# arielgabizon/barretenberg

Hardware: AMD Instinct MI355X
Metric: BN254 G1 MSM points/sec at n=2^20 (Fr NTT elems/sec in 'ntt') (higher is better)
Workload: dtype u32x9 (256-bit Montgomery, 29-bit limbs)

## Files before the change

barretenberg_amd/csrc/msm.hip:

```cpp
#include <hip/hip_runtime.h>

#include <algorithm>
#include <mutex>
#include <stdint.h>
#include <stdio.h>
#include <stdlib.h>
#include <string.h>
#include <vector>

#include "bbgpu_internal.h"
#include "g1.hpp"
#include "g1_quad.hpp"
#include "host_g1.hpp"

namespace bbgpu {

using Fr = FrP;
#define FRONT_PRIO() __builtin_amdgcn_s_setprio(2)
constexpr int TAIL_PRIO = 3;
constexpr int SCALAR_BITS = 254;
constexpr int MSM_MAX_C = 16;
constexpr int MSM_THREADS = 256;

__device__ __forceinline__ void ld8(const uint32_t* p, uint32_t (&w)[8])
{
    const uint4* q = reinterpret_cast<const uint4*>(p);
    uint4 a = q[0], b = q[1];
    w[0] = a.x; w[1] = a.y; w[2] = a.z; w[3] = a.w;
    w[4] = b.x; w[5] = b.y; w[6] = b.z; w[7] = b.w;
}
__device__ __forceinline__ void ld16(const uint32_t* p, uint32_t (&w)[16])
{
    const uint4* q = reinterpret_cast<const uint4*>(p);
#pragma unroll
    for (int i = 0; i < 4; i++) {
        uint4 a = q[i];
        w[4 * i] = a.x; w[4 * i + 1] = a.y; w[4 * i + 2] = a.z; w[4 * i + 3] = a.w;
    }
}
__device__ __forceinline__ void st32(uint32_t* p, const uint32_t (&w)[32])
{
    uint4* q = reinterpret_cast<uint4*>(p);
#pragma unroll
    for (int i = 0; i < 8; i++) q[i] = make_uint4(w[4 * i], w[4 * i + 1], w[4 * i + 2], w[4 * i + 3]);
}
__device__ __forceinline__ void ld32(const uint32_t* p, uint32_t (&w)[32])
{
    const uint4* q = reinterpret_cast<const uint4*>(p);
#pragma unroll
    for (int i = 0; i < 8; i++) {
        uint4 a = q[i];
        w[4 * i] = a.x; w[4 * i + 1] = a.y; w[4 * i + 2] = a.z; w[4 * i + 3] = a.w;
    }
}

struct WinLayout {
    uint16_t off[66];
};
static WinLayout make_layout(int c, bool balanced)
{
    WinLayout LO{};
    const int W = msm_num_windows(c);
    if (!balanced) {
        for (int w = 0; w <= W; w++) LO.off[w] = (uint16_t)(c * w);
        return LO;
    }
    const int base = SCALAR_BITS / W, rem = SCALAR_BITS - base * W;
    int bit = 0;
    for (int w = 0; w < W; w++) {
        LO.off[w] = (uint16_t)bit;
        bit += base + (w < rem ? 1 : 0);
    }
    LO.off[W] = (uint16_t)bit;
    return LO;
}
__global__ void srs_convert_kernel(const uint32_t* __restrict__ table, uint32_t* __restrict__ srs, uint32_t n, uint32_t stride_words)
{
    const uint32_t i = blockIdx.x * blockDim.x + threadIdx.x;
    if (i >= n) return;
    uint32_t w[16];
    ld16(table + (size_t)i * stride_words, w);
    AffineV<2> a;
    load_affine_m256(a, w);
    uint32_t o[16];
    store_affine_m261(o, a.x, a.y);
    uint4* q = reinterpret_cast<uint4*>(srs + (size_t)i * 16);
#pragma unroll
    for (int k = 0; k < 4; k++) q[k] = make_uint4(o[4 * k], o[4 * k + 1], o[4 * k + 2], o[4 * k + 3]);
}

__global__ void srs_export_kernel(const uint32_t* __restrict__ srs, uint32_t* __restrict__ table, uint32_t n)
{
    const uint32_t i = blockIdx.x * blockDim.x + threadIdx.x;
    if (i >= n) return;
    uint32_t w[16];
    ld16(srs + (size_t)i * 16, w);
    AffineV<1> a;
    load_affine_m261(a, w);
    uint32_t o[8];
    uint32_t* dst = table + (size_t)i * 32;
    to_canonical(m261_to_m256<Fq>(a.x), o);
    for (int k = 0; k < 8; k++) dst[k] = o[k];
    to_canonical(m261_to_m256<Fq>(a.y), o);
    for (int k = 0; k < 8; k++) dst[8 + k] = o[k];
    auto bx = mul(a.x, fe_from<Fq>(Fq::BETA));
    to_canonical(m261_to_m256<Fq>(bx), o);
    for (int k = 0; k < 8; k++) dst[16 + k] = o[k];
    to_canonical(m261_to_m256<Fq>(weak(neg(a.y))), o);
// ... 116 lines not shown
    } else {
        return dg[i];
    }
}
template <class DT> __device__ __forceinline__ void load_digits8(const DT* __restrict__ dg, const unsigned long long* __restrict__ sg, uint32_t i8, int (&d)[8])
{
    const uint4 q = *reinterpret_cast<const uint4*>(dg + i8);
    const uint32_t w[4] = { q.x, q.y, q.z, q.w };
    if constexpr (DigitTraits<DT>::wide) {
        const uint32_t sb = reinterpret_cast<const uint8_t*>(sg)[i8 >> 3];
#pragma unroll
        for (int k = 0; k < 8; k++) {
            const int u = (int)((w[k >> 1] >> (16 * (k & 1))) & 0xffffu);
            d[k] = ((sb >> k) & 1u) ? -u - 1 : u;
        }
    } else {
#pragma unroll
        for (int k = 0; k < 8; k++) d[k] = (int)(int16_t)(w[k >> 1] >> (16 * (k & 1)));
    }
}
template <class DT> __global__ void __launch_bounds__(MSM_THREADS) msm_digits_kernel(ScalarSets sets, DT* __restrict__ digits_all, unsigned long long* __restrict__ signs_all,
                                                               uint32_t n, WinLayout LO, uint32_t num_windows, uint32_t wb, uint32_t we)
{
    FRONT_PRIO();
    const uint32_t i = blockIdx.x * blockDim.x + threadIdx.x;
    if (i >= n) return;
    const uint32_t* __restrict__ scalars = sets.p[blockIdx.y];
    DT* __restrict__ digits = digits_all + (size_t)blockIdx.y * num_windows * n;
    const uint32_t s64 = (n + 63) >> 6;
    unsigned long long* __restrict__ signs = signs_all + (size_t)blockIdx.y * num_windows * s64;
    uint32_t w[8], k[9];
    ld8(scalars + (size_t)i * 8, w);
    to_canonical(exact_limbs(mul(unpack<Fr>(w), fe_from<Fr>(Fr::M256_TO_PLAIN))), w);
#pragma unroll
    for (int j = 0; j < 8; j++) k[j] = w[j];
    k[8] = 0;
    uint32_t carry = 0;
    for (uint32_t win = 0; win < we; win++) {
        const uint32_t bit = LO.off[win], sz = LO.off[win + 1] - bit, j = bit >> 5, s = bit & 31;
        const uint32_t half = 1u << (sz - 1), mask = (1u << sz) - 1;
        uint32_t v = 0;
        if (j < 8) {
            v = k[j] >> s;
            if (s + sz > 32) v |= k[j + 1] << (32 - s);
        }
        v = (v & mask) + carry;
        carry = (win + 1 < num_windows && v >= half) ? 1u : 0u;
        const int32_t d = (int32_t)v - (int32_t)(carry << sz);
        if (win >= wb) {
            if constexpr (DigitTraits<DT>::wide) {
                const unsigned long long neg = __ballot(d < 0);
                digits[(size_t)win * n + i] = (DT)(d < 0 ? -d - 1 : d);
                if ((threadIdx.x & 63u) == 0) signs[(size_t)win * s64 + (i >> 6)] = neg;
            } else {
                digits[(size_t)win * n + i] = (DT)d;
            }
        }
    }
}

constexpr int SORT_THREADS = 1024;
constexpr uint32_t SORT_MAX_LB = 7;
constexpr uint32_t SORTB_MAX_PARTS = 8;
constexpr uint32_t SORTB_SPLIT_MIN = 1u << 16;

__device__ __forceinline__ bool wave_keys_heavy(bool valid, uint32_t key)
{
    const uint64_t vm = __ballot(valid);
    if (!vm) return false;
    const uint32_t k0 = __builtin_amdgcn_readlane(key, __ffsll((unsigned long long)vm) - 1);
    return 4 * __popcll(__ballot(valid && key == k0)) >= __popcll(vm);
}
__device__ __forceinline__ uint32_t lds_inc_dedup(uint32_t* ctr, uint32_t key, bool heavy)
{
    if (!heavy) return atomicAdd(&ctr[key], 1u);
    const uint32_t lane = __lane_id();
    uint64_t todo = __ballot(1);
    uint32_t res = 0;
    for (int it = 0; it < 4 && todo; it++) {
        const int leader = __ffsll((unsigned long long)todo) - 1;
        const uint32_t kk = __builtin_amdgcn_readlane(key, leader);
// ... 50 lines not shown
    }
    __syncthreads();
    if (threadIdx.x < bins) histA[((size_t)wl * slices + s) * bins + threadIdx.x] = lh[threadIdx.x];
}

__global__ void __launch_bounds__(SORT_THREADS) sortA_colscan_kernel(uint32_t* __restrict__ histA, uint32_t* __restrict__ bintot, uint32_t bins,
                                                                   uint32_t slices)
{
    FRONT_PRIO();
    const uint32_t wl = blockIdx.y, lane = threadIdx.x & 63;
    const uint32_t bin = blockIdx.x * (SORT_THREADS / 64) + (threadIdx.x >> 6);
    if (bin >= bins) return;
    uint32_t* H = histA + (size_t)wl * slices * bins + bin;
    const uint32_t spp = (slices + 63) / 64;
    const uint32_t s0 = min(slices, lane * spp), s1 = min(slices, s0 + spp);
    uint32_t sum = 0;
    for (uint32_t s = s0; s < s1; s++) sum += H[(size_t)s * bins];
    uint32_t incl = sum;
#pragma unroll
    for (int off = 1; off < 64; off <<= 1) {
        const uint32_t v = __shfl_up(incl, off);
        if ((int)lane >= off) incl += v;
    }
    uint32_t run = incl - sum;
    for (uint32_t s = s0; s < s1; s++) {
        const uint32_t cnt = H[(size_t)s * bins];
        H[(size_t)s * bins] = run;
        run += cnt;
    }
    if (lane == 63) bintot[(size_t)wl * bins + bin] = incl;
}
__global__ void __launch_bounds__(SORT_THREADS) sortA_scan_kernel(const uint32_t* __restrict__ bintot, uint32_t* __restrict__ binstart,
                                                                uint32_t* __restrict__ totals, uint32_t bins, uint32_t* __restrict__ solo_bases,
                                                                uint32_t* __restrict__ solo_gstart_end)
{
    FRONT_PRIO();
    __shared__ uint32_t part[SORT_THREADS];
    const uint32_t wl = blockIdx.x, t = threadIdx.x;
    const uint32_t mine = t < bins ? bintot[(size_t)wl * bins + t] : 0;
    part[t] = mine;
    __syncthreads();
    for (uint32_t off = 1; off < SORT_THREADS; off <<= 1) {
        uint32_t v = t >= off ? part[t - off] : 0;
        __syncthreads();
        part[t] += v;
        __syncthreads();
    }
    if (t < bins) binstart[(size_t)wl * bins + t] = part[t] - mine;
    if (t == SORT_THREADS - 1) {
        totals[wl] = part[SORT_THREADS - 1];
        if (solo_bases) {
            solo_bases[0] = 0;
            solo_bases[1] = part[SORT_THREADS - 1];
            solo_gstart_end[0] = part[SORT_THREADS - 1];
            solo_gstart_end[1] = 0xffffffffu;
        }
    }
}
__global__ void sort_bases_kernel(const uint32_t* __restrict__ totals, uint32_t* __restrict__ bases, uint32_t* __restrict__ gstart_end, uint32_t nw)
{
    FRONT_PRIO();
    if (threadIdx.x == 0 && blockIdx.x == 0) {
        uint32_t run = 0;
        for (uint32_t w = 0; w < nw; w++) {
            bases[w] = run;
            run += totals[w];
        }
        bases[nw] = run;
        gstart_end[0] = run;
        gstart_end[1] = 0xffffffffu;
    }
}


template <class DT> __global__ void __launch_bounds__(SORT_THREADS) __attribute__((amdgpu_num_vgpr(32))) sortA_scatter_kernel(const DT* __restrict__ digits, const unsigned long long* __restrict__ signs, const uint32_t* __restrict__ cursorsA,
                                                                   const uint32_t* __restrict__ binstart, const uint32_t* __restrict__ bases,
                                                                   uint32_t* __restrict__ tmp, uint32_t n, uint32_t bins, uint32_t lb,
                                                                   uint32_t slices, uint32_t slice_len, uint32_t win0, uint32_t wpg,
                                                                   uint32_t idx_stride, uint32_t windows_per_job, uint32_t first_i0, uint32_t last_i1, uint32_t blo, uint32_t bcnt)
{
    FRONT_PRIO();
    __shared__ uint32_t lc[SORT_THREADS];
    const uint32_t s = blockIdx.x, wl = blockIdx.y;
    if (threadIdx.x < bins)
        lc[threadIdx.x] = cursorsA[((size_t)wl * slices + s) * bins + threadIdx.x] + binstart[(size_t)wl * bins + threadIdx.x] + bases[wl];
    __syncthreads();
    const uint32_t lo = s * slice_len, hi = min(n, lo + slice_len);
    const uint32_t lomask = (1u << lb) - 1;
    const uint32_t s64 = (n + 63) >> 6;
    if ((n & 7u) == 0) {
        const uint32_t lo8 = lo & ~7u, bpw = lo < hi ? (((hi + 7u) & ~7u) - lo8) >> 3 : 0u;
        for (uint32_t u = threadIdx.x; u < wpg * bpw; u += SORT_THREADS) {
            const uint32_t k = u / bpw, i8 = lo8 + (u - k * bpw) * 8;
            const uint32_t wabs = win0 + wl * wpg + k;
            const uint32_t row = (wabs % windows_per_job) * idx_stride;
            const uint32_t klo = (k == 0) ? max(lo, first_i0) : lo, khi = (k + 1 == wpg) ? min(hi, last_i1) : hi;
            int d[8];
            load_digits8<DT>(digits + (size_t)wabs * n, signs + (size_t)wabs * s64, i8, d);
#pragma unroll
            for (int j = 0; j < 8; j++) {
                if (d[j] && i8 + j >= klo && i8 + j < khi) {
                    const uint32_t b = (uint32_t)((d[j] < 0 ? -d[j] : d[j]) - 1);
                    if (b - blo < bcnt) {
// ... 289 lines not shown
    const u32x4* q = reinterpret_cast<const u32x4*>(p);
    r.q0 = q[0]; r.q1 = q[1]; r.q2 = q[2]; r.q3 = q[3];
#endif
}
__device__ __forceinline__ void row_land(RowRegs& r, uint32_t (&w)[16])
{
#if defined(__HIP_DEVICE_COMPILE__)
    __builtin_amdgcn_s_waitcnt(0x0f70);
    asm volatile("" : "+v"(r.q0), "+v"(r.q1), "+v"(r.q2), "+v"(r.q3));
#endif
#pragma unroll
    for (int i = 0; i < 4; i++) { w[i] = r.q0[i]; w[4 + i] = r.q1[i]; w[8 + i] = r.q2[i]; w[12 + i] = r.q3[i]; }
}
__device__ __forceinline__ void value_landed(uint32_t& v)
{
#if defined(__HIP_DEVICE_COMPILE__)
    asm volatile("" : "+v"(v));
#endif
}
__device__ __forceinline__ void operand_done(Fe<Fq, 1, 1>& x, Fe<Fq, 1, 2>& y)
{
#if defined(__HIP_DEVICE_COMPILE__)
    asm volatile("" : "+v"(x.d[0]), "+v"(x.d[1]), "+v"(x.d[2]), "+v"(x.d[3]), "+v"(x.d[4]), "+v"(x.d[5]), "+v"(x.d[6]), "+v"(x.d[7]), "+v"(x.d[8]));
    asm volatile("" : "+v"(y.d[0]), "+v"(y.d[1]), "+v"(y.d[2]), "+v"(y.d[3]), "+v"(y.d[4]), "+v"(y.d[5]), "+v"(y.d[6]), "+v"(y.d[7]), "+v"(y.d[8]));
#endif
}
constexpr int RAW_WORDS = 4 * NL;
constexpr uint32_t HEAVY_WGS = 256;
constexpr uint32_t HEAVY_IDS = 1 + HEAVY_WGS;
static_assert(MSM_THREADS == (int)HEAVY_WGS, "heavy-bucket queue header is cleared / combined by one lane per K4h workgroup");

__global__ void __launch_bounds__(MSM_THREADS) msm_accumulate_kernel(const uint32_t* __restrict__ srs, const uint32_t* __restrict__ sorted,
                                                                   const uint32_t* __restrict__ gstart, uint32_t* __restrict__ partials,
                                                                   uint32_t total_buckets, uint32_t ch, uint32_t prio, uint32_t* __restrict__ heavy_counter)
{
    if (heavy_counter && blockIdx.x == 0) {
        heavy_counter[threadIdx.x] = 0;
        if (threadIdx.x == 0) heavy_counter[MSM_THREADS] = 0;
    }
    if (prio == 1) __builtin_amdgcn_s_setprio(1);
    else if (prio == 2) __builtin_amdgcn_s_setprio(2);
    const uint32_t t = blockIdx.x * blockDim.x + threadIdx.x;
    const uint32_t M = gstart[total_buckets];
    const uint32_t p0 = t * ch;
    if (p0 >= M) return;
    const uint32_t p1 = min(M, p0 + ch);
    uint32_t lo = 0, hi = total_buckets;
    while (hi - lo > 1) {
        const uint32_t mid = (lo + hi) >> 1;
        if (gstart[mid] <= p0) lo = mid; else hi = mid;
    }
    uint32_t b = lo;
    uint32_t next_end = gstart[b + 1];
    Xyzz acc;
    set_infinity(acc);
    uint32_t after_next = gstart[min(b + 2, total_buckets + 1)];
    bool acc_inf = true;
    uint32_t v = sorted[p0];
    uint32_t vn = sorted[p0 + 1 < p1 ? p0 + 1 : p0];
    RowRegs row;
    uint32_t w[16];
    row_request(row, srs + (size_t)(v & 0x7fffffffu) * 16);
    Fe<Fq, 1, 1> px;
    Fe<Fq, 1, 2> py;
    row_land(row, w);
    load_affine_m261_signed(px, py, w, (v >> 31) != 0);
    operand_done(px, py);
    row_request(row, srs + (size_t)(vn & 0x7fffffffu) * 16);
    uint32_t e = p0;
    uint32_t trips = ch;
    do {
        const uint32_t vnn = sorted[min(e + 2, p1 - 1)];
        const bool start = (e == next_end) || acc_inf;
        if (start) {
            if (e == next_end) {
                store_raw(partials + (size_t)(b + t) * RAW_WORDS, acc);
// ... 47 lines not shown
}
#define TAIL_OCC __attribute__((amdgpu_waves_per_eu(4, 4)))
constexpr int FOLD_T = 256;
constexpr int FOLD_LDS_WORDS = (FOLD_T / 2) * RAW_WORDS;
__device__ __forceinline__ void wg_tree_sum(Xyzz& acc, uint32_t* sh, uint32_t T, uint32_t t)
{
    constexpr uint32_t STRIDE = FOLD_T / 2;
    for (uint32_t half = T >> 1; half >= 1; half >>= 1) {
        if (t >= half && t < 2 * half) {
#pragma unroll
            for (int i = 0; i < NL; i++) {
                sh[(0 * NL + i) * STRIDE + t - half] = acc.x.d[i];
                sh[(1 * NL + i) * STRIDE + t - half] = acc.y.d[i];
                sh[(2 * NL + i) * STRIDE + t - half] = acc.zz.d[i];
                sh[(3 * NL + i) * STRIDE + t - half] = acc.zzz.d[i];
            }
        }
        __syncthreads();
        if (t < half) {
            Xyzz q, r;
#pragma unroll
            for (int i = 0; i < NL; i++) {
                q.x.d[i] = sh[(0 * NL + i) * STRIDE + t];
                q.y.d[i] = sh[(1 * NL + i) * STRIDE + t];
                q.zz.d[i] = sh[(2 * NL + i) * STRIDE + t];
                q.zzz.d[i] = sh[(3 * NL + i) * STRIDE + t];
            }
            add(r, acc, q);
            acc = r;
        }
        __syncthreads();
    }
}
__global__ void __launch_bounds__(MSM_THREADS) TAIL_OCC msm_merge_kernel(const uint32_t* __restrict__ gstart, const uint32_t* __restrict__ partials,
                                                              uint32_t* __restrict__ buckets, uint32_t* __restrict__ heavy, uint32_t bucket_begin, uint32_t total_buckets,
                                                              uint32_t ch, uint32_t MERGE_LIGHT, uint32_t logG)
{
    __builtin_amdgcn_s_setprio(TAIL_PRIO);
    const uint32_t t = blockIdx.x * blockDim.x + threadIdx.x;
    const uint32_t G = 1u << logG, b = bucket_begin + (t >> logG), j = t & (G - 1);
    if (b >= total_buckets) return;
    const uint32_t s = gstart[b], e = gstart[b + 1];
    Xyzz acc;
    set_infinity(acc);
    if (e > s) {
        const uint32_t t0 = s / ch, t1 = (e - 1) / ch;
        if (t1 - t0 >= MERGE_LIGHT) {
            if (j == 0) heavy[HEAVY_IDS + atomicAdd(&heavy[0], 1u)] = b;
            return;
        }
        for (uint32_t k = t0 + j; k <= t1; k += G) {
            Xyzz q, r;
            load_raw(q, partials + (size_t)(b + k) * RAW_WORDS);
            add(r, acc, q);
            acc = r;
        }
    }
    for (uint32_t off = G >> 1; off >= 1; off >>= 1) {
        const Xyzz o = shfl_down_xyzz(acc, off);
        if (j < off) {
            Xyzz r;
            add(r, acc, o);
            acc = r;
        }
    }
    if (j == 0) {
        uint32_t o[32];
        store_xyzz(o, acc);
        st32(buckets + (size_t)b * 32, o);
    }
}
__global__ void __launch_bounds__(MSM_THREADS) TAIL_OCC msm_merge_heavy_kernel(const uint32_t* __restrict__ gstart, const uint32_t* __restrict__ partials,
                                                                    uint32_t* __restrict__ buckets, uint32_t* __restrict__ heavy, uint32_t ch, uint32_t* __restrict__ hpart)
{
    __builtin_amdgcn_s_setprio(TAIL_PRIO);
    __shared__ uint32_t sh[FOLD_LDS_WORDS];
    __shared__ uint32_t last_flag;
    const uint32_t count = heavy[0];
    const uint32_t K = count ? gridDim.x / count : 0;
    if (K < 2) {
        for (uint32_t item = blockIdx.x; item < count; item += gridDim.x) {
            const uint32_t b = heavy[HEAVY_IDS + item];
            const uint32_t s = gstart[b], e = gstart[b + 1];
            const uint32_t t0 = s / ch, t1 = (e - 1) / ch;
            Xyzz acc;
            set_infinity(acc);
            for (uint32_t t = t0 + threadIdx.x; t <= t1; t += MSM_THREADS) {
                Xyzz q, r;
                load_raw(q, partials + (size_t)(b + t) * RAW_WORDS);
                add(r, acc, q);
                acc = r;
            }
            __syncthreads();
            wg_tree_sum(acc, sh, MSM_THREADS, threadIdx.x);
            if (threadIdx.x == 0) {
                uint32_t o[32];
                store_xyzz(o, acc);
                st32(buckets + (size_t)b * 32, o);
            }
        }
        return;
    }
    const uint32_t item = blockIdx.x / K, sub = blockIdx.x - item * K;
    if (item >= count) return;
    const uint32_t b = heavy[HEAVY_IDS + item];
    const uint32_t s = gstart[b], e = gstart[b + 1];
    const uint32_t t0 = s / ch, t1 = (e - 1) / ch, total = t1 - t0 + 1;
// ... 57 lines not shown
    constexpr uint32_t NW = T / 64;
    const uint32_t waves = min(NW, (active + 15) / 16);
    if (waves <= 1) return acc;
    if (lane < 4) {
#pragma unroll
        for (int i = 0; i < NL; i++) sh[(wave * 4 + l) * NL + i] = acc.d[i];
    }
    __syncthreads();
    if (wave == 0) {
        acc = quad_zero();
        if (qd < NW) {
#pragma unroll
            for (int i = 0; i < NL; i++) acc.d[i] = sh[(qd * 4 + l) * NL + i];
        }
        for (uint32_t off = NW >> 1; off >= 1; off >>= 1) {
            if (off >= waves) continue;
            FqN o;
#pragma unroll
            for (int i = 0; i < NL; i++) o.d[i] = __shfl_down(acc.d[i], off * 4);
            if (qd < off) acc = quad_add(acc, o, l);
        }
    }
    return acc;
}
__device__ __forceinline__ void quad_store8(uint32_t* dst8, const uint32_t (&w)[8])
{
    uint4* q = reinterpret_cast<uint4*>(dst8);
    q[0] = make_uint4(w[0], w[1], w[2], w[3]);
    q[1] = make_uint4(w[4], w[5], w[6], w[7]);
}

__global__ void __launch_bounds__(MSM_THREADS) TAIL_OCC msm_merge_quad_kernel(const uint32_t* __restrict__ gstart, const uint32_t* __restrict__ partials,
                                                                   uint32_t* __restrict__ buckets, uint32_t* __restrict__ heavy, uint32_t bucket_begin, uint32_t total_buckets,
                                                                   uint32_t ch, uint32_t MERGE_LIGHT, uint32_t logQ)
{
    __builtin_amdgcn_s_setprio(TAIL_PRIO);
    const uint32_t t = blockIdx.x * blockDim.x + threadIdx.x, l = t & 3, quad = t >> 2;
    const uint32_t Q = 1u << logQ, b = bucket_begin + (quad >> logQ), j = quad & (Q - 1);
    if (b >= total_buckets) return;
    const uint32_t s = gstart[b], e = gstart[b + 1];
    FqN acc = quad_zero();
    if (e > s) {
        const uint32_t t0 = s / ch, t1 = (e - 1) / ch;
        if (t1 - t0 >= MERGE_LIGHT) {
            if (j == 0 && l == 0) heavy[HEAVY_IDS + atomicAdd(&heavy[0], 1u)] = b;
            return;
        }
        uint32_t k = t0 + j;
        if (k <= t1) {
            const uint32_t* src = partials + (size_t)(b + k) * RAW_WORDS + NL * l;
#pragma unroll
            for (int i = 0; i < NL; i++) acc.d[i] = src[i];
            FqN q = quad_zero();
            k += Q;
            if (k <= t1) {
                src = partials + (size_t)(b + k) * RAW_WORDS + NL * l;
#pragma unroll
                for (int i = 0; i < NL; i++) q.d[i] = src[i];
            }
            while (k <= t1) {
                FqN qn = quad_zero();
                const uint32_t kn = k + Q;
                if (kn <= t1) {
                    src = partials + (size_t)(b + kn) * RAW_WORDS + NL * l;
#pragma unroll
                    for (int i = 0; i < NL; i++) qn.d[i] = src[i];
                }
                acc = quad_add(acc, q, l);
                q = qn;
                k = kn;
            }
        }
    }
// ... 102 lines not shown
        quad_store8((row ? R + ((size_t)g * H + idx) * 32 : Cc + ((size_t)g * L + idx) * 32) + 8 * l, w);
    }
}
__global__ void __launch_bounds__(QFOLD_T) TAIL_OCC msm_final_quad_kernel(const uint32_t* __restrict__ R, const uint32_t* __restrict__ Cc, uint32_t* __restrict__ out,
                                                                 uint32_t hbits, uint32_t lbits)
{
    __builtin_amdgcn_s_setprio(TAIL_PRIO);
    __shared__ uint32_t sh[(QFOLD_T / 64) * 4 * NL];
    const uint32_t g = blockIdx.y, t = threadIdx.x, job = blockIdx.x, l = t & 3, quad = t >> 2;
    const uint32_t H = 1u << hbits, L = 1u << lbits;
    const uint32_t* src;
    uint32_t count, slot, k = 0;
    bool sliced = true;
    if (job == 0) { src = R + (size_t)g * H * 32; count = H; slot = 0; sliced = false; }
    else if (job < 1 + hbits) { k = job - 1; src = R + (size_t)g * H * 32; count = H >> 1; slot = 1 + k; }
    else { k = job - 1 - hbits; src = Cc + (size_t)g * L * 32; count = L >> 1; slot = 32 + k; }
    FqN acc = quad_zero();
    bool first = true;
    for (uint32_t e = quad; e < count; e += QFOLD_T / 4) {
        const FqN v = quad_load(src + (size_t)(sliced ? insert_one_bit(e, k) : e) * 32, l);
        acc = first ? v : quad_add(acc, v, l);
        first = false;
    }
    acc = block_quad_sum(acc, sh, t, min(count, (uint32_t)QFOLD_T / 4));
    if (t < 4) {
        uint32_t w[8];
        to_canonical(m261_to_m256<Fq>(acc), w);
        quad_store8(out + ((size_t)g * 64 + slot) * 32 + 8 * l, w);
    }
}

int msm_choose_c(size_t n)
{
    int lg = 0;
    while (((size_t)1 << lg) < n) lg++;
    int c = lg - 4;
    if (c < 4) c = 4;
    if (c > MSM_MAX_C) c = MSM_MAX_C;
    return c;
}
int msm_num_windows(int c)
{
    return SCALAR_BITS / c + 1;
}

struct MsmPlan {
    uint32_t n, c, W, nb, hbits, lbits, slices, slice_len, sort_lb, sort_bins;
};
constexpr uint32_t ACC_WG_PER_CU = 3;
static uint32_t acc_capacity_lanes()
{
    static const uint32_t lanes = [] {
        int dev = 0, cus = 256;
        (void)hipGetDevice(&dev);
        (void)hipDeviceGetAttribute(&cus, hipDeviceAttributeMultiprocessorCount, dev);
        return (uint32_t)cus * ACC_WG_PER_CU * MSM_THREADS;
    }();
    return lanes;
}
constexpr uint32_t MIN_CHUNK = 8;
constexpr uint64_t TINY_ENTRIES = (uint64_t)1 << 16;
constexpr uint32_t TINY_MIN_CHUNK = 4;
static uint32_t min_chunk(uint64_t m) { return m <= TINY_ENTRIES ? TINY_MIN_CHUNK : MIN_CHUNK; }
static uint32_t chunk_len_m(const uint64_t m)
{
    static const double step[3] = { 6.4, 9.2, 13.4 };
    const uint64_t per_k = (uint64_t)acc_capacity_lanes() / ACC_WG_PER_CU;
    uint32_t best = 0;
    double best_cost = 0.0;
    for (uint32_t k = 1; k <= ACC_WG_PER_CU; k++) {
        const uint32_t ch = std::max<uint32_t>(min_chunk(m), (uint32_t)((m + per_k * k - 1) / (per_k * k)));
        const double cost = ch * step[k - 1];
        if (!best || cost < best_cost) { best = ch; best_cost = cost; }
    }
    return best;
}
static uint32_t chunk_len(size_t n, uint32_t nw)
{
    return chunk_len_m((uint64_t)n * nw);
}
static size_t arena_points(const MsmPlan& P, uint32_t nw)
{
    const size_t H = (size_t)1 << P.hbits, L = (size_t)1 << P.lbits;
    return (size_t)nw * (H + L) + 64;
}
static bool rowcol_two_step(const MsmPlan& P)
{
    return P.hbits + P.lbits >= 15;
}
static size_t seg_points(const MsmPlan& P, uint32_t nw)
{
    const size_t H = (size_t)1 << P.hbits, L = (size_t)1 << P.lbits;
    return rowcol_two_step(P) ? (size_t)nw * 2 * (H * L / ROWCOL_SEG) : 0;
}
static MsmPlan make_plan(size_t n, int c)
{
    MsmPlan P;
    P.n = (uint32_t)n;
    P.c = (uint32_t)c;
    P.W = (uint32_t)msm_num_windows(c);
    P.nb = 1u << (c - 1);
    P.lbits = (c - 1) / 2;
    P.hbits = (c - 1) - P.lbits;
    P.slices = std::max<uint32_t>(1, 512 / P.W);
    P.sort_lb = std::min<uint32_t>(SORT_MAX_LB, (uint32_t)c - 1);
    P.sort_bins = P.nb >> P.sort_lb;
    if ((uint64_t)P.slices * 4096 > n) P.slices = std::max<uint32_t>(1, (uint32_t)(n / 4096));
    P.slice_len = (uint32_t)((n + P.slices - 1) / P.slices);
    return P;
}

struct MsmCarve {
    size_t digits, signs, histA, histB, binstart, bintot, tmp_entries, gstart, totals, heavy, sorted, partials, buckets, arena, segs, end;
    size_t chunks_cap, histB_bytes;
};
static MsmCarve carve(const MsmPlan& P, size_t n, size_t nw, size_t ng)
{
    auto al = [](size_t x) { return (x + 255) & ~(size_t)255; };
    MsmCarve L;
    size_t p = 0;
    const size_t wmax = std::max<size_t>(P.W, nw);
    L.digits = p;      p += al(wmax * n * 2);
    L.signs = p;       p += al(wmax * ((n + 63) / 64) * 8);
    L.histA = p;       p += al(nw * P.slices * 1024 * 4);
    L.histB_bytes = (uint64_t)n * nw >= ((uint64_t)1 << 21) ? (size_t)MSM_MAX_JOBS * 1024 * SORTB_MAX_PARTS * 128 * 4 : 0;
    L.histB = p;       p += al(L.histB_bytes);
    L.binstart = p;    p += al(nw * 1024 * 4 + 256);
    L.bintot = p;      p += al(nw * 1024 * 4 + 256);
    L.tmp_entries = p; p += al(nw * n * 4);
    L.gstart = p;      p += al((ng * P.nb + 2) * 4);
    L.totals = p;      p += al(nw * 8 + 512);
    L.heavy = p;       p += al((ng * P.nb + HEAVY_IDS) * 4 + 256 + (size_t)HEAVY_WGS * RAW_WORDS * 4);
    L.sorted = p;      p += al(nw * n * 4);
    L.chunks_cap = (n * nw + min_chunk(n * nw) - 1) / min_chunk(n * nw) + 1;
    L.partials = p;    p += al((ng * P.nb + L.chunks_cap) * RAW_WORDS * 4);
    L.buckets = p;     p += al(ng * P.nb * 128);
    L.arena = p;       p += al(arena_points(P, (uint32_t)ng) * 128);
    L.segs = p;        p += al(seg_points(P, (uint32_t)ng) * 128);
    L.end = p;
    return L;
}
size_t MsmWorkspace::bytes_needed(size_t n, int c, int nw, int ng)
{
    return carve(make_plan(n, c), n, (size_t)nw, (size_t)(ng > 0 ? ng : nw)).end;
}

int MsmWorkspace::ensure(size_t bytes)
{
    if (bytes <= cap) return BBGPU_OK;
    if (base) (void)dev_free(base);
    base = nullptr;
    cap = 0;
    HIPCHK(dev_malloc((void**)&base, bytes));
    cap = bytes;
    return BBGPU_OK;
}
void MsmWorkspace::release()
{
    if (base) (void)dev_free(base);
    if (h_out) (void)hipHostFree(h_out);
    base = nullptr;
    h_out = nullptr;
    cap = 0;
}

int msm_issue_rows(MsmSlot& S, const uint32_t* d_srs, const uint32_t* d_tab, size_t tab_stride, int tab_c, const uint64_t* d_scalars, size_t n,
                   uint64_t row_begin, uint64_t row_end, hipStream_t st, int want_timing)
// ... 120 lines not shown
    unsigned long long* signs = (unsigned long long*)(p + LY.signs);
    uint32_t* histA = (uint32_t*)(p + LY.histA);
    uint32_t* histB = (uint32_t*)(p + LY.histB);
    uint32_t* binstart = (uint32_t*)(p + LY.binstart);
    uint32_t* bintot = (uint32_t*)(p + LY.bintot);
    uint32_t* tmp_entries = (uint32_t*)(p + LY.tmp_entries);
    uint32_t* gstart = (uint32_t*)(p + LY.gstart);
    uint32_t* totals = (uint32_t*)(p + LY.totals);
    uint32_t* bases = totals + nw;
    uint32_t* heavy = (uint32_t*)(p + LY.heavy);
    uint32_t* sorted = (uint32_t*)(p + LY.sorted);
    uint32_t* partials = (uint32_t*)(p + LY.partials);
    uint32_t* buckets = (uint32_t*)(p + LY.buckets);
    uint32_t* scratch = (uint32_t*)(p + LY.arena);
    if ((uint64_t)G * slices * sort_bins > (uint64_t)nw * P.slices * 1024 || sort_bins > 1024 ||
        (size_t)G * ((size_t)(1u << P.hbits) + (size_t)(1u << P.lbits)) + 64 > arena_points(P, G)) {
        set_error("internal: MSM launch shape exceeds the workspace layout");
        return BBGPU_ERR_STATE;
    }

    hipEvent_t* ev = S.ev;
    const bool tm = want_timing == 1, tm_acc = want_timing != 0;
    S.timed_light = want_timing == 2;
    if (tm_acc) {
        if (!S.ev[0])
            for (int i = 0; i < 8; i++) HIPCHK(hipEventCreate(&S.ev[i]));
        if (tm) HIPCHK(hipEventRecord(ev[0], st));
        S.timed = true;
    }

    if (bshare) {
        HIPCHK(hipMemsetAsync(scratch, 0, (size_t)G * BH * 128, st));
    }
    ScalarSets sets{};
    for (int j = 0; j < jobs; j++) sets.p[j] = (const uint32_t*)d_scalars_v[j];
    const bool wide = c > 16;
    if (wide) msm_digits_kernel<uint16_t><<<dim3((P.n + MSM_THREADS - 1) / MSM_THREADS, jobs), MSM_THREADS, 0, st>>>(sets, (uint16_t*)digits, signs, P.n, make_layout(c, table), P.W, (uint32_t)wb, (uint32_t)we);
    else msm_digits_kernel<int16_t><<<dim3((P.n + MSM_THREADS - 1) / MSM_THREADS, jobs), MSM_THREADS, 0, st>>>(sets, (int16_t*)digits, signs, P.n, make_layout(c, table), P.W, (uint32_t)wb, (uint32_t)we);
    if (tm) HIPCHK(hipEventRecord(ev[1], st));
    if (wide) sortA_hist_kernel<uint16_t><<<dim3(slices, G), SORT_THREADS, 0, st>>>((const uint16_t*)digits, signs, histA, P.n, sort_bins, sort_lb, slices, slice_len, (uint32_t)wb, wpg, row_i0, row_i1, blo, bcnt);
    else sortA_hist_kernel<int16_t><<<dim3(slices, G), SORT_THREADS, 0, st>>>((const int16_t*)digits, signs, histA, P.n, sort_bins, sort_lb, slices, slice_len, (uint32_t)wb, wpg, row_i0, row_i1, blo, bcnt);
    sortA_colscan_kernel<<<dim3((sort_bins + SORT_THREADS / 64 - 1) / (SORT_THREADS / 64), G), SORT_THREADS, 0, st>>>(histA, bintot, sort_bins, slices);
    sortA_scan_kernel<<<G, SORT_THREADS, 0, st>>>(bintot, binstart, totals, sort_bins, G == 1 ? bases : nullptr, gstart + (size_t)G * P.nb);
    if (G > 1) sort_bases_kernel<<<1, 64, 0, st>>>(totals, bases, gstart + (size_t)G * P.nb, G);
    if ((P.n & 7u) == 0) {
        if (wide) sortA_scatter_staged_kernel<uint16_t><<<dim3(slices, G), SORT_THREADS, 0, st>>>((const uint16_t*)digits, signs, histA, binstart, bases, tmp_entries, P.n, sort_bins, sort_lb, slices,
                                                                                  slice_len, (uint32_t)wb, wpg, idx_stride, P.W, row_i0, row_i1, blo, bcnt);
        else sortA_scatter_staged_kernel<int16_t><<<dim3(slices, G), SORT_THREADS, 0, st>>>((const int16_t*)digits, signs, histA, binstart, bases, tmp_entries, P.n, sort_bins, sort_lb, slices,
                                                                            slice_len, (uint32_t)wb, wpg, idx_stride, P.W, row_i0, row_i1, blo, bcnt);
    } else if (wide) sortA_scatter_kernel<uint16_t><<<dim3(slices, G), SORT_THREADS, 0, st>>>((const uint16_t*)digits, signs, histA, binstart, bases, tmp_entries, P.n, sort_bins, sort_lb, slices,
                                                                   slice_len, (uint32_t)wb, wpg, idx_stride, P.W, row_i0, row_i1, blo, bcnt);
    else sortA_scatter_kernel<int16_t><<<dim3(slices, G), SORT_THREADS, 0, st>>>((const int16_t*)digits, signs, histA, binstart, bases, tmp_entries, P.n, sort_bins, sort_lb, slices,
                                                                   slice_len, (uint32_t)wb, wpg, idx_stride, P.W, row_i0, row_i1, blo, bcnt);
    if (table) {
        uint32_t parts = ((uint64_t)n * nw1 >= ((uint64_t)1 << 21) && G <= MSM_MAX_JOBS) ? SORTB_MAX_PARTS : 1u;
        if ((size_t)G * sort_bins * parts * 128 * 4 > LY.histB_bytes) parts = 1;
        if (parts > 1) sortB_count_kernel<SORT_THREADS><<<dim3(sort_bins, G, parts), SORT_THREADS, 0, st>>>(tmp_entries, binstart, bases, histB, sort_bins, parts);
        sortB_staged_kernel<SORT_THREADS><<<dim3(sort_bins, G, parts), SORT_THREADS, 0, st>>>(tmp_entries, binstart, bases, sorted, gstart, sort_bins, sort_lb, P.nb, histB, parts);
    } else sortB_staged_kernel<256><<<dim3(sort_bins, G), 256, 0, st>>>(tmp_entries, binstart, bases, sorted, gstart, sort_bins, sort_lb, P.nb, nullptr, 1u);
    if (tm_acc) HIPCHK(hipEventRecord(ev[2], st));
    const uint32_t total_buckets = G * P.nb;
    const uint64_t m_expected = bshare ? std::max<uint64_t>(1, (uint64_t)n * nw * bcnt / P.nb) : (uint64_t)n * nw;
    const uint32_t merge_buckets = bshare ? bcnt : total_buckets;
    const bool tp = hint && jobs == 1;
    constexpr uint32_t TP_MIN_CHUNK = 20;
    uint32_t ch = bshare ? chunk_len_m(m_expected) : chunk_len(n, nw);
    ch = std::max(ch, min_chunk((uint64_t)n * nw));
    if (tp && ch < TP_MIN_CHUNK)
        ch = std::max(ch, std::min<uint32_t>(TP_MIN_CHUNK, (uint32_t)(m_expected / (acc_capacity_lanes() / ACC_WG_PER_CU))));
    const uint32_t avg_partials = (uint32_t)(m_expected / ((uint64_t)merge_buckets * ch)) + 1;
    uint32_t logG = 0;
    while ((1u << logG) < avg_partials && logG < 6 && ((uint64_t)merge_buckets << (logG + 1)) <= ((uint64_t)1 << 16)) logG++;
    const uint32_t merge_light = std::max(6u, 8u << logG);
    const uint32_t max_chunks = (uint32_t)(((uint64_t)n * nw + ch - 1) / ch);
    msm_accumulate_kernel<<<(max_chunks + MSM_THREADS - 1) / MSM_THREADS, MSM_THREADS, 0, st>>>(points, sorted, gstart, partials, total_buckets, ch, 0, heavy);
    if (tm_acc) {
        HIPCHK(hipEventRecord(ev[3], st));
        if (int rc = acc_ring_record(S, st)) return rc;
    } else {
        S.acc_seq = 0;
    }
    if ((uint64_t)n * nw <= ((uint64_t)1 << 21)) {
        uint32_t logQ = 0;
        while ((2u << logQ) < avg_partials && logQ < 4 && ((uint64_t)merge_buckets << (logQ + 3)) <= ((uint64_t)1 << 17)) logQ++;
        msm_merge_quad_kernel<<<(uint32_t)((((uint64_t)merge_buckets << (logQ + 2)) + MSM_THREADS - 1) / MSM_THREADS), MSM_THREADS, 0, st>>>(gstart, partials, buckets, heavy, blo, blo + merge_buckets, ch,
                                                                                                                                  std::max(32u, 8u << logQ), logQ);
    } else msm_merge_kernel<<<(uint32_t)((((uint64_t)merge_buckets << logG) + MSM_THREADS - 1) / MSM_THREADS), MSM_THREADS, 0, st>>>(gstart, partials, buckets, heavy,
                                                                                                                     blo, blo + merge_buckets, ch, merge_light, logG);
    msm_merge_heavy_kernel<<<HEAVY_WGS, MSM_THREADS, 0, st>>>(gstart, partials, buckets, heavy, ch, heavy + (((size_t)G * P.nb + HEAVY_IDS + 63) & ~(size_t)63));
    if (tm) HIPCHK(hipEventRecord(ev[4], st));

    const uint32_t H = 1u << P.hbits, L = 1u << P.lbits;
    {
        uint32_t* Rr = scratch;
        uint32_t* Cc = scratch + (size_t)G * H * 32;
        uint32_t* const dest = (uint32_t*)ws.h_out + (size_t)PC.hout_group * 64 * 32;
        const uint32_t zero_words = G * 64 * 32;
        if (!bshare && rowcol_two_step(P) && (tp || jobs > 1)) {
            uint32_t* segs = (uint32_t*)(p + LY.segs);
            const uint32_t seg_lanes = 2 * (H * L / ROWCOL_SEG);
            msm_rowcol_seg_kernel<<<dim3((seg_lanes + MSM_THREADS - 1) / MSM_THREADS, G), MSM_THREADS, 0, st>>>(buckets, segs, H, L, dest, zero_words);
            msm_segsum_quad_kernel<<<dim3(H + L, G), 64, 0, st>>>(segs, Rr, Cc, H, L);
        } else msm_rowcol_quad_kernel<<<dim3((bshare ? brow1 - brow0 : H) + L, G), QFOLD_T, 0, st>>>(buckets, Rr, Cc, H, L, dest, zero_words, bshare ? brow0 : 0u,
                                                                                                  bshare ? brow1 - brow0 : H);
        if (tm) HIPCHK(hipEventRecord(ev[5], st));
        msm_final_quad_kernel<<<dim3(1 + P.hbits + P.lbits, G), QFOLD_T, 0, st>>>(Rr, Cc, dest, P.hbits, P.lbits);
        if (tm) HIPCHK(hipEventRecord(ev[6], st));
    }
    HIPCHK(hipEventRecord(S.done, st));
    HIPCHK(launch_check());
    S.npieces++;
    S.pending = true;
    return BBGPU_OK;
}

static host::Xyzz group_sum(const MsmSlot& S, const MsmPiece& PC, uint32_t w)
{
    auto pt = [&](uint32_t slot) {
        host::Xyzz q;
        memcpy(&q, (const uint8_t*)S.ws.h_out + ((size_t)(PC.hout_group + w) * 64 + slot) * 128, 128);
        return q;
    };
// ... 166 lines not shown
```

Before: 950.4 million.

## Fold scalars above r/2 and pick accumulate chunk length on device

Scalars larger than half the group order are replaced by r−k, with their signed window digits negated, so digit magnitudes and top-window occupancy shrink. The accumulate chunk length is now computed on the device from the actual sorted entry count M, clamped between the minimum and the host choice. It is stored next to gstart and read by the accumulate and merge kernels, which tries to spread work evenly over all launched lanes when fewer entries survive than expected. Helpers move into a new header, and extra asm barriers make the merge kernels load the chunk value at runtime.

Result: no change. 950.4 million (-0.0%).

```diff
diff --git a/barretenberg_amd/csrc/msm.hip b/barretenberg_amd/csrc/msm.hip
--- a/barretenberg_amd/csrc/msm.hip
+++ b/barretenberg_amd/csrc/msm.hip
@@ -12,15 +12,13 @@
 #include "g1.hpp"
 #include "g1_quad.hpp"
 #include "host_g1.hpp"
+#include "msm_chunks.hpp"
 
 namespace bbgpu {
 
 using Fr = FrP;
 #define FRONT_PRIO() __builtin_amdgcn_s_setprio(2)
 constexpr int TAIL_PRIO = 3;
-constexpr int SCALAR_BITS = 254;
-constexpr int MSM_MAX_C = 16;
-constexpr int MSM_THREADS = 256;
 
 __device__ __forceinline__ void ld8(const uint32_t* p, uint32_t (&w)[8])
 {
@@ -54,26 +52,6 @@
     }
 }
 
-struct WinLayout {
-    uint16_t off[66];
-};
-static WinLayout make_layout(int c, bool balanced)
-{
-    WinLayout LO{};
-    const int W = msm_num_windows(c);
-    if (!balanced) {
-        for (int w = 0; w <= W; w++) LO.off[w] = (uint16_t)(c * w);
-        return LO;
-    }
-    const int base = SCALAR_BITS / W, rem = SCALAR_BITS - base * W;
-    int bit = 0;
-    for (int w = 0; w < W; w++) {
-        LO.off[w] = (uint16_t)bit;
-        bit += base + (w < rem ? 1 : 0);
-    }
-    LO.off[W] = (uint16_t)bit;
-    return LO;
-}
 __global__ void srs_convert_kernel(const uint32_t* __restrict__ table, uint32_t* __restrict__ srs, uint32_t n, uint32_t stride_words)
 {
     const uint32_t i = blockIdx.x * blockDim.x + threadIdx.x;
@@ -256,21 +234,13 @@
     uint32_t w[8], k[9];
     ld8(scalars + (size_t)i * 8, w);
     to_canonical(exact_limbs(mul(unpack<Fr>(w), fe_from<Fr>(Fr::M256_TO_PLAIN))), w);
+    const uint32_t fold = msm_fold_scalar(w);
 #pragma unroll
     for (int j = 0; j < 8; j++) k[j] = w[j];
     k[8] = 0;
     uint32_t carry = 0;
     for (uint32_t win = 0; win < we; win++) {
-        const uint32_t bit = LO.off[win], sz = LO.off[win + 1] - bit, j = bit >> 5, s = bit & 31;
-        const uint32_t half = 1u << (sz - 1), mask = (1u << sz) - 1;
-        uint32_t v = 0;
-        if (j < 8) {
-            v = k[j] >> s;
-            if (s + sz > 32) v |= k[j + 1] << (32 - s);
-        }
-        v = (v & mask) + carry;
-        carry = (win + 1 < num_windows && v >= half) ? 1u : 0u;
-        const int32_t d = (int32_t)v - (int32_t)(carry << sz);
+        const int32_t d = msm_window_digit(k, LO, win, num_windows, fold, carry);
         if (win >= wb) {
             if constexpr (DigitTraits<DT>::wide) {
                 const unsigned long long neg = __ballot(d < 0);
@@ -387,7 +357,7 @@
 }
 __global__ void __launch_bounds__(SORT_THREADS) sortA_scan_kernel(const uint32_t* __restrict__ bintot, uint32_t* __restrict__ binstart,
                                                                 uint32_t* __restrict__ totals, uint32_t bins, uint32_t* __restrict__ solo_bases,
-                                                                uint32_t* __restrict__ solo_gstart_end)
+                                                                uint32_t* __restrict__ solo_gstart_end, ChunkArgs CA)
 {
     FRONT_PRIO();
     __shared__ uint32_t part[SORT_THREADS];
@@ -409,10 +379,11 @@
             solo_bases[1] = part[SORT_THREADS - 1];
             solo_gstart_end[0] = part[SORT_THREADS - 1];
             solo_gstart_end[1] = 0xffffffffu;
-        }
-    }
-}
-__global__ void sort_bases_kernel(const uint32_t* __restrict__ totals, uint32_t* __restrict__ bases, uint32_t* __restrict__ gstart_end, uint32_t nw)
+            solo_gstart_end[2] = msm_chunk_choice(part[SORT_THREADS - 1], CA.lanes, CA.ch_min, CA.ch_host, 0).ch;
+        }
+    }
+}
+__global__ void sort_bases_kernel(const uint32_t* __restrict__ totals, uint32_t* __restrict__ bases, uint32_t* __restrict__ gstart_end, uint32_t nw, ChunkArgs CA)
 {
     FRONT_PRIO();
     if (threadIdx.x == 0 && blockIdx.x == 0) {
@@ -424,6 +395,7 @@
         bases[nw] = run;
         gstart_end[0] = run;
         gstart_end[1] = 0xffffffffu;
+        gstart_end[2] = msm_chunk_choice(run, CA.lanes, CA.ch_min, CA.ch_host, 0).ch;
     }
 }
 
@@ -779,7 +751,7 @@
 
 __global__ void __launch_bounds__(MSM_THREADS) msm_accumulate_kernel(const uint32_t* __restrict__ srs, const uint32_t* __restrict__ sorted,
                                                                    const uint32_t* __restrict__ gstart, uint32_t* __restrict__ partials,
-                                                                   uint32_t total_buckets, uint32_t ch, uint32_t prio, uint32_t* __restrict__ heavy_counter)
+                                                                   uint32_t total_buckets, uint32_t prio, uint32_t* __restrict__ heavy_counter)
 {
     if (heavy_counter && blockIdx.x == 0) {
         heavy_counter[threadIdx.x] = 0;
@@ -789,6 +761,7 @@
     else if (prio == 2) __builtin_amdgcn_s_setprio(2);
     const uint32_t t = blockIdx.x * blockDim.x + threadIdx.x;
     const uint32_t M = gstart[total_buckets];
+    const uint32_t ch = __builtin_amdgcn_readfirstlane(gstart[total_buckets + 2]);
     const uint32_t p0 = t * ch;
     if (p0 >= M) return;
     const uint32_t p1 = min(M, p0 + ch);
@@ -902,15 +875,30 @@
         __syncthreads();
     }
 }
+__device__ __forceinline__ uint32_t merge_chunk_len(const uint32_t* __restrict__ ch_dev)
+{
+    uint32_t zero = 0;
+#if defined(__HIP_DEVICE_COMPILE__)
+    asm("" : "+v"(zero));
+#endif
+    return ch_dev[zero];
+}
+__device__ __forceinline__ void bounds_and_chunk_landed(uint32_t& s, uint32_t& e, uint32_t& ch)
+{
+#if defined(__HIP_DEVICE_COMPILE__)
+    asm volatile("" : "+v"(s), "+v"(e), "+v"(ch));
+#endif
+}
 __global__ void __launch_bounds__(MSM_THREADS) TAIL_OCC msm_merge_kernel(const uint32_t* __restrict__ gstart, const uint32_t* __restrict__ partials,
                                                               uint32_t* __restrict__ buckets, uint32_t* __restrict__ heavy, uint32_t bucket_begin, uint32_t total_buckets,
-                                                              uint32_t ch, uint32_t MERGE_LIGHT, uint32_t logG)
+                                                              const uint32_t* __restrict__ ch_dev, uint32_t MERGE_LIGHT, uint32_t logG)
 {
     __builtin_amdgcn_s_setprio(TAIL_PRIO);
     const uint32_t t = blockIdx.x * blockDim.x + threadIdx.x;
     const uint32_t G = 1u << logG, b = bucket_begin + (t >> logG), j = t & (G - 1);
     if (b >= total_buckets) return;
-    const uint32_t s = gstart[b], e = gstart[b + 1];
+    uint32_t s = gstart[b], e = gstart[b + 1], ch = merge_chunk_len(ch_dev);
+    bounds_and_chunk_landed(s, e, ch);
     Xyzz acc;
     set_infinity(acc);
     if (e > s) {
@@ -941,8 +929,9 @@
     }
 }
 __global__ void __launch_bounds__(MSM_THREADS) TAIL_OCC msm_merge_heavy_kernel(const uint32_t* __restrict__ gstart, const uint32_t* __restrict__ partials,
-                                                                    uint32_t* __restrict__ buckets, uint32_t* __restrict__ heavy, uint32_t ch, uint32_t* __restrict__ hpart)
-{
+                                                                    uint32_t* __restrict__ buckets, uint32_t* __restrict__ heavy, const uint32_t* __restrict__ ch_dev, uint32_t* __restrict__ hpart)
+{
+    const uint32_t ch = __builtin_amdgcn_readfirstlane(*ch_dev);
     __builtin_amdgcn_s_setprio(TAIL_PRIO);
     __shared__ uint32_t sh[FOLD_LDS_WORDS];
     __shared__ uint32_t last_flag;
@@ -1066,13 +1055,14 @@
 
 __global__ void __launch_bounds__(MSM_THREADS) TAIL_OCC msm_merge_quad_kernel(const uint32_t* __restrict__ gstart, const uint32_t* __restrict__ partials,
                                                                    uint32_t* __restrict__ buckets, uint32_t* __restrict__ heavy, uint32_t bucket_begin, uint32_t total_buckets,
-                                                                   uint32_t ch, uint32_t MERGE_LIGHT, uint32_t logQ)
+                                                                   const uint32_t* __restrict__ ch_dev, uint32_t MERGE_LIGHT, uint32_t logQ)
 {
     __builtin_amdgcn_s_setprio(TAIL_PRIO);
     const uint32_t t = blockIdx.x * blockDim.x + threadIdx.x, l = t & 3, quad = t >> 2;
     const uint32_t Q = 1u << logQ, b = bucket_begin + (quad >> logQ), j = quad & (Q - 1);
     if (b >= total_buckets) return;
-    const uint32_t s = gstart[b], e = gstart[b + 1];
+    uint32_t s = gstart[b], e = gstart[b + 1], ch = merge_chunk_len(ch_dev);
+    bounds_and_chunk_landed(s, e, ch);
     FqN acc = quad_zero();
     if (e > s) {
         const uint32_t t0 = s / ch, t1 = (e - 1) / ch;
@@ -1241,22 +1231,16 @@
 
 int msm_choose_c(size_t n)
 {
-    int lg = 0;
-    while (((size_t)1 << lg) < n) lg++;
-    int c = lg - 4;
-    if (c < 4) c = 4;
-    if (c > MSM_MAX_C) c = MSM_MAX_C;
-    return c;
+    return msm_window_bits_of(n);
 }
 int msm_num_windows(int c)
 {
-    return SCALAR_BITS / c + 1;
+    return msm_windows_of(c);
 }
 
 struct MsmPlan {
     uint32_t n, c, W, nb, hbits, lbits, slices, slice_len, sort_lb, sort_bins;
 };
-constexpr uint32_t ACC_WG_PER_CU = 3;
 static uint32_t acc_capacity_lanes()
 {
     static const uint32_t lanes = [] {
@@ -1267,22 +1251,9 @@
     }();
     return lanes;
 }
-constexpr uint32_t MIN_CHUNK = 8;
-constexpr uint64_t TINY_ENTRIES = (uint64_t)1 << 16;
-constexpr uint32_t TINY_MIN_CHUNK = 4;
-static uint32_t min_chunk(uint64_t m) { return m <= TINY_ENTRIES ? TINY_MIN_CHUNK : MIN_CHUNK; }
 static uint32_t chunk_len_m(const uint64_t m)
 {
-    static const double step[3] = { 6.4, 9.2, 13.4 };
-    const uint64_t per_k = (uint64_t)acc_capacity_lanes() / ACC_WG_PER_CU;
-    uint32_t best = 0;
-    double best_cost = 0.0;
-    for (uint32_t k = 1; k <= ACC_WG_PER_CU; k++) {
-        const uint32_t ch = std::max<uint32_t>(min_chunk(m), (uint32_t)((m + per_k * k - 1) / (per_k * k)));
-        const double cost = ch * step[k - 1];
-        if (!best || cost < best_cost) { best = ch; best_cost = cost; }
-    }
-    return best;
+    return chunk_len_for(m, acc_capacity_lanes());
 }
 static uint32_t chunk_len(size_t n, uint32_t nw)
 {
@@ -1337,11 +1308,11 @@
     L.binstart = p;    p += al(nw * 1024 * 4 + 256);
     L.bintot = p;      p += al(nw * 1024 * 4 + 256);
     L.tmp_entries = p; p += al(nw * n * 4);
-    L.gstart = p;      p += al((ng * P.nb + 2) * 4);
+    L.gstart = p;      p += al((ng * P.nb + 3) * 4);
     L.totals = p;      p += al(nw * 8 + 512);
     L.heavy = p;       p += al((ng * P.nb + HEAVY_IDS) * 4 + 256 + (size_t)HEAVY_WGS * RAW_WORDS * 4);
     L.sorted = p;      p += al(nw * n * 4);
-    L.chunks_cap = (n * nw + min_chunk(n * nw) - 1) / min_chunk(n * nw) + 1;
+    L.chunks_cap = chunks_cap_for((uint64_t)n * nw);
     L.partials = p;    p += al((ng * P.nb + L.chunks_cap) * RAW_WORDS * 4);
     L.buckets = p;     p += al(ng * P.nb * 128);
     L.arena = p;       p += al(arena_points(P, (uint32_t)ng) * 128);
@@ -1528,6 +1499,21 @@
     if (bshare) {
         HIPCHK(hipMemsetAsync(scratch, 0, (size_t)G * BH * 128, st));
     }
+    const uint32_t total_buckets = G * P.nb;
+    const uint64_t m_expected = bshare ? std::max<uint64_t>(1, (uint64_t)n * nw * bcnt / P.nb) : (uint64_t)n * nw;
+    const uint32_t merge_buckets = bshare ? bcnt : total_buckets;
+    const bool tp = hint && jobs == 1;
+    constexpr uint32_t TP_MIN_CHUNK = 20;
+    const uint32_t ch_min = min_chunk((uint64_t)n * nw);
+    uint32_t ch = bshare ? chunk_len_m(m_expected) : chunk_len(n, nw);
+    ch = std::max(ch, ch_min);
+    if (tp && ch < TP_MIN_CHUNK)
+        ch = std::max(ch, std::min<uint32_t>(TP_MIN_CHUNK, (uint32_t)(m_expected / (acc_capacity_lanes() / ACC_WG_PER_CU))));
+    const uint32_t max_chunks = (uint32_t)(((uint64_t)n * nw + ch - 1) / ch);
+    const uint32_t acc_grid = (max_chunks + MSM_THREADS - 1) / MSM_THREADS;
+    const bool full_list = !bshare && row_i0 == 0 && row_i1 == n && wb == 0 && we == (int)P.W;
+    const ChunkArgs chunk_args{ acc_grid * (uint32_t)MSM_THREADS, full_list ? ch_min : ch, ch };
+    uint32_t* const ch_dev = gstart + (size_t)total_buckets + 2;
     ScalarSets sets{};
     for (int j = 0; j < jobs; j++) sets.p[j] = (const uint32_t*)d_scalars_v[j];
     const bool wide = c > 16;
@@ -1537,8 +1523,8 @@
     if (wide) sortA_hist_kernel<uint16_t><<<dim3(slices, G), SORT_THREADS, 0, st>>>((const uint16_t*)digits, signs, histA, P.n, sort_bins, sort_lb, slices, slice_len, (uint32_t)wb, wpg, row_i0, row_i1, blo, bcnt);
     else sortA_hist_kernel<int16_t><<<dim3(slices, G), SORT_THREADS, 0, st>>>((const int16_t*)digits, signs, histA, P.n, sort_bins, sort_lb, slices, slice_len, (uint32_t)wb, wpg, row_i0, row_i1, blo, bcnt);
     sortA_colscan_kernel<<<dim3((sort_bins + SORT_THREADS / 64 - 1) / (SORT_THREADS / 64), G), SORT_THREADS, 0, st>>>(histA, bintot, sort_bins, slices);
-    sortA_scan_kernel<<<G, SORT_THREADS, 0, st>>>(bintot, binstart, totals, sort_bins, G == 1 ? bases : nullptr, gstart + (size_t)G * P.nb);
-    if (G > 1) sort_bases_kernel<<<1, 64, 0, st>>>(totals, bases, gstart + (size_t)G * P.nb, G);
+    sortA_scan_kernel<<<G, SORT_THREADS, 0, st>>>(bintot, binstart, totals, sort_bins, G == 1 ? bases : nullptr, gstart + (size_t)G * P.nb, chunk_args);
+    if (G > 1) sort_bases_kernel<<<1, 64, 0, st>>>(totals, bases, gstart + (size_t)G * P.nb, G, chunk_args);
     if ((P.n & 7u) == 0) {
         if (wide) sortA_scatter_staged_kernel<uint16_t><<<dim3(slices, G), SORT_THREADS, 0, st>>>((const uint16_t*)digits, signs, histA, binstart, bases, tmp_entries, P.n, sort_bins, sort_lb, slices,
                                                                                   slice_len, (uint32_t)wb, wpg, idx_stride, P.W, row_i0, row_i1, blo, bcnt);
@@ -1555,21 +1541,11 @@
         sortB_staged_kernel<SORT_THREADS><<<dim3(sort_bins, G, parts), SORT_THREADS, 0, st>>>(tmp_entries, binstart, bases, sorted, gstart, sort_bins, sort_lb, P.nb, histB, parts);
     } else sortB_staged_kernel<256><<<dim3(sort_bins, G), 256, 0, st>>>(tmp_entries, binstart, bases, sorted, gstart, sort_bins, sort_lb, P.nb, nullptr, 1u);
     if (tm_acc) HIPCHK(hipEventRecord(ev[2], st));
-    const uint32_t total_buckets = G * P.nb;
-    const uint64_t m_expected = bshare ? std::max<uint64_t>(1, (uint64_t)n * nw * bcnt / P.nb) : (uint64_t)n * nw;
-    const uint32_t merge_buckets = bshare ? bcnt : total_buckets;
-    const bool tp = hint && jobs == 1;
-    constexpr uint32_t TP_MIN_CHUNK = 20;
-    uint32_t ch = bshare ? chunk_len_m(m_expected) : chunk_len(n, nw);
-    ch = std::max(ch, min_chunk((uint64_t)n * nw));
-    if (tp && ch < TP_MIN_CHUNK)
-        ch = std::max(ch, std::min<uint32_t>(TP_MIN_CHUNK, (uint32_t)(m_expected / (acc_capacity_lanes() / ACC_WG_PER_CU))));
     const uint32_t avg_partials = (uint32_t)(m_expected / ((uint64_t)merge_buckets * ch)) + 1;
     uint32_t logG = 0;
     while ((1u << logG) < avg_partials && logG < 6 && ((uint64_t)merge_buckets << (logG + 1)) <= ((uint64_t)1 << 16)) logG++;
     const uint32_t merge_light = std::max(6u, 8u << logG);
-    const uint32_t max_chunks = (uint32_t)(((uint64_t)n * nw + ch - 1) / ch);
-    msm_accumulate_kernel<<<(max_chunks + MSM_THREADS - 1) / MSM_THREADS, MSM_THREADS, 0, st>>>(points, sorted, gstart, partials, total_buckets, ch, 0, heavy);
+    msm_accumulate_kernel<<<acc_grid, MSM_THREADS, 0, st>>>(points, sorted, gstart, partials, total_buckets, 0, heavy);
     if (tm_acc) {
         HIPCHK(hipEventRecord(ev[3], st));
         if (int rc = acc_ring_record(S, st)) return rc;
@@ -1579,11 +1555,11 @@
     if ((uint64_t)n * nw <= ((uint64_t)1 << 21)) {
         uint32_t logQ = 0;
         while ((2u << logQ) < avg_partials && logQ < 4 && ((uint64_t)merge_buckets << (logQ + 3)) <= ((uint64_t)1 << 17)) logQ++;
-        msm_merge_quad_kernel<<<(uint32_t)((((uint64_t)merge_buckets << (logQ + 2)) + MSM_THREADS - 1) / MSM_THREADS), MSM_THREADS, 0, st>>>(gstart, partials, buckets, heavy, blo, blo + merge_buckets, ch,
+        msm_merge_quad_kernel<<<(uint32_t)((((uint64_t)merge_buckets << (logQ + 2)) + MSM_THREADS - 1) / MSM_THREADS), MSM_THREADS, 0, st>>>(gstart, partials, buckets, heavy, blo, blo + merge_buckets, ch_dev,
                                                                                                                                   std::max(32u, 8u << logQ), logQ);
     } else msm_merge_kernel<<<(uint32_t)((((uint64_t)merge_buckets << logG) + MSM_THREADS - 1) / MSM_THREADS), MSM_THREADS, 0, st>>>(gstart, partials, buckets, heavy,
-                                                                                                                     blo, blo + merge_buckets, ch, merge_light, logG);
-    msm_merge_heavy_kernel<<<HEAVY_WGS, MSM_THREADS, 0, st>>>(gstart, partials, buckets, heavy, ch, heavy + (((size_t)G * P.nb + HEAVY_IDS + 63) & ~(size_t)63));
+                                                                                                                     blo, blo + merge_buckets, ch_dev, merge_light, logG);
+    msm_merge_heavy_kernel<<<HEAVY_WGS, MSM_THREADS, 0, st>>>(gstart, partials, buckets, heavy, ch_dev, heavy + (((size_t)G * P.nb + HEAVY_IDS + 63) & ~(size_t)63));
     if (tm) HIPCHK(hipEventRecord(ev[4], st));
 
     const uint32_t H = 1u << P.hbits, L = 1u << P.lbits;
diff --git a/barretenberg_amd/csrc/msm_chunks.hpp b/barretenberg_amd/csrc/msm_chunks.hpp
--- /dev/null
+++ b/barretenberg_amd/csrc/msm_chunks.hpp
@@ -0,0 +1,131 @@
+#pragma once
+#include <stddef.h>
+#include <stdint.h>
+
+#include "bn254_params.h"
+#include "fe.hpp"
+
+namespace bbgpu {
+
+constexpr int SCALAR_BITS = 254;
+constexpr int MSM_MAX_C = 16;
+constexpr int MSM_THREADS = 256;
+
+inline int msm_windows_of(int c)
+{
+    return SCALAR_BITS / c + 1;
+}
+inline int msm_window_bits_of(size_t n)
+{
+    int lg = 0;
+    while (((size_t)1 << lg) < n) lg++;
+    int c = lg - 4;
+    if (c < 4) c = 4;
+    if (c > MSM_MAX_C) c = MSM_MAX_C;
+    return c;
+}
+struct WinLayout {
+    uint16_t off[66];
+};
+inline WinLayout make_layout(int c, bool balanced)
+{
+    WinLayout LO{};
+    const int W = msm_windows_of(c);
+    if (!balanced) {
+        for (int w = 0; w <= W; w++) LO.off[w] = (uint16_t)(c * w);
+        return LO;
+    }
+    const int base = SCALAR_BITS / W, rem = SCALAR_BITS - base * W;
+    int bit = 0;
+    for (int w = 0; w < W; w++) {
+        LO.off[w] = (uint16_t)bit;
+        bit += base + (w < rem ? 1 : 0);
+    }
+    LO.off[W] = (uint16_t)bit;
+    return LO;
+}
+
+BB_HD constexpr uint64_t fr_half64(int i)
+{
+    return (FrP::P64[i] >> 1) | (i < 3 ? FrP::P64[i + 1] << 63 : 0ull);
+}
+BB_HD uint32_t sub_borrow32(uint32_t a, uint32_t b, bool& borrow)
+{
+    uint32_t t, r;
+    const bool o1 = __builtin_sub_overflow(a, b, &t), o2 = __builtin_sub_overflow(t, (uint32_t)borrow, &r);
+    borrow = o1 | o2;
+    return r;
+}
+BB_HD uint32_t msm_fold_scalar(uint32_t (&k)[8])
+{
+    bool fold = false;
+#pragma unroll
+    for (int i = 0; i < 8; i++)
+        (void)sub_borrow32((uint32_t)((i & 1) ? fr_half64(i >> 1) >> 32 : fr_half64(i >> 1)), k[i], fold);
+    bool b = false;
+#pragma unroll
+    for (int i = 0; i < 8; i++) {
+        const uint32_t t = sub_borrow32((uint32_t)((i & 1) ? FrP::P64[i >> 1] >> 32 : FrP::P64[i >> 1]), k[i], b);
+        k[i] = fold ? t : k[i];
+    }
+    return fold ? 1u : 0u;
+}
+BB_HD int32_t msm_window_digit(const uint32_t (&k)[9], const WinLayout& LO, uint32_t win, uint32_t num_windows, uint32_t fold, uint32_t& carry)
+{
+    const uint32_t bit = LO.off[win], sz = LO.off[win + 1] - bit, j = bit >> 5, s = bit & 31;
+    const uint32_t half = 1u << (sz - 1), mask = (1u << sz) - 1;
+    uint32_t v = 0;
+    if (j < 8) {
+        v = k[j] >> s;
+        if (s + sz > 32) v |= k[j + 1] << (32 - s);
+    }
+    v = (v & mask) + carry;
+    carry = (win + 1 < num_windows && v >= half + fold) ? 1u : 0u;
+    const int32_t d = (int32_t)v - (int32_t)(carry << sz);
+    const int32_t m = -(int32_t)fold;
+    return (d ^ m) - m;
+}
+
+constexpr uint32_t MIN_CHUNK = 8;
+constexpr uint64_t TINY_ENTRIES = (uint64_t)1 << 16;
+constexpr uint32_t TINY_MIN_CHUNK = 4;
+constexpr uint32_t ACC_WG_PER_CU = 3;
+inline uint32_t min_chunk(uint64_t m) { return m <= TINY_ENTRIES ? TINY_MIN_CHUNK : MIN_CHUNK; }
+inline uint32_t chunk_len_for(const uint64_t m, const uint64_t capacity_lanes)
+{
+    static const double step[3] = { 6.4, 9.2, 13.4 };
+    const uint64_t per_k = capacity_lanes / ACC_WG_PER_CU;
+    uint32_t best = 0;
+    double best_cost = 0.0;
+    for (uint32_t k = 1; k <= ACC_WG_PER_CU; k++) {
+        const uint32_t mc = min_chunk(m), by_lanes = (uint32_t)((m + per_k * k - 1) / (per_k * k));
+        const uint32_t ch = mc > by_lanes ? mc : by_lanes;
+        const double cost = ch * step[k - 1];
+        if (!best || cost < best_cost) { best = ch; best_cost = cost; }
+    }
+    return best;
+}
+inline size_t chunks_cap_for(uint64_t entries_max)
+{
+    return (size_t)((entries_max + min_chunk(entries_max) - 1) / min_chunk(entries_max) + 1);
+}
+struct ChunkArgs {
+    uint32_t lanes, ch_min, ch_host;
+};
+struct ChunkChoice {
+    uint32_t ch, chunks;
+    uint64_t slot_end;
+};
+BB_HD ChunkChoice msm_chunk_choice(uint32_t M, uint32_t lanes, uint32_t ch_min, uint32_t ch_host, uint32_t total_buckets)
+{
+    ChunkChoice c;
+    uint32_t ch = M / lanes + (M % lanes ? 1u : 0u);
+    if (ch < ch_min) ch = ch_min;
+    if (ch > ch_host) ch = ch_host;
+    c.ch = ch;
+    c.chunks = M / ch + (M % ch ? 1u : 0u);
+    c.slot_end = (uint64_t)total_buckets + c.chunks;
+    return c;
+}
+
+}
```
